# JuliaControl/ModelPredictiveControl.jl

Measured on AMD Instinct MI355X. Metric: QP solves/sec (moveinput!), higher is better.
Workload: dtype f64

## Files before the change

### modelpredictivecontrol.jl_amd/csrc/mpcqp_bodies.h

```cpp
#pragma once
#include <math.h>

#include <type_traits>

#include "mpcqp_types.h"

#if defined(MPCQP_PROFILE) && defined(__HIP_DEVICE_COMPILE__)
#define MPCQP_TIC() const long long tic_ = clock64()
#define MPCQP_TOC(i) prof_[i] += (double)(clock64() - tic_)
#define MPCQP_TICK(name) const long long name = clock64()
#define MPCQP_TOCK(i, name) prof_[i] += (double)(clock64() - name)
#elif defined(MPCQP_ISA_MARKERS) && defined(__HIP_DEVICE_COMPILE__)
#define MPCQP_MARK_(txt) do { __builtin_amdgcn_sched_barrier(0); asm volatile("; MPCQP_MARK " txt ::: "memory"); __builtin_amdgcn_sched_barrier(0); } while (0)
#define MPCQP_TIC() MPCQP_MARK_("tic")
#define MPCQP_TOC(i) MPCQP_MARK_("toc " #i)
#define MPCQP_TICK(name) MPCQP_MARK_("tic " #name)
#define MPCQP_TOCK(i, name) MPCQP_MARK_("toc " #i)
#define MPCQP_MTIC() MPCQP_MARK_("tic")
#define MPCQP_MTOC(name) MPCQP_MARK_("toc " name)
#else
#define MPCQP_TIC() ((void)0)
#define MPCQP_TOC(i) ((void)0)
#define MPCQP_TICK(name) ((void)0)
#define MPCQP_TOCK(i, name) ((void)0)
#endif
#ifndef MPCQP_MTIC
#define MPCQP_MTIC() ((void)0)
#define MPCQP_MTOC(name) ((void)0)
#endif

#ifndef MPCQP_POLISH_FACTS
#define MPCQP_POLISH_FACTS 1
#endif
#ifndef MPCQP_POLISH_BUDGET
#define MPCQP_POLISH_BUDGET 3
#endif
#ifndef MPCQP_POLISH_MU
#define MPCQP_POLISH_MU 1e-7
#endif
#ifndef MPCQP_POLISH_RP
#define MPCQP_POLISH_RP 1e-6
#endif
#ifndef MPCQP_EAPPLY44_HCMAX
#define MPCQP_EAPPLY44_HCMAX 10
#endif
#ifndef MPCQP_EAPPLY44_UNROLL
#define MPCQP_EAPPLY44_UNROLL 2
#endif
#ifndef MPCQP_EV_UNROLL
#if defined(MPCQP_STEP_WAVES) && MPCQP_STEP_WAVES == 1
#define MPCQP_EV_UNROLL 16
#else
#define MPCQP_EV_UNROLL 4
#endif
#endif
#define MPCQP_PRAGMA_(x) _Pragma(#x)
#define MPCQP_PRAGMA(x) MPCQP_PRAGMA_(x)
#ifndef MPCQP_ETDE_UNROLL
#if defined(MPCQP_STEP_WAVES) && MPCQP_STEP_WAVES == 1
#define MPCQP_ETDE_UNROLL 4
#else
#define MPCQP_ETDE_UNROLL 2
#endif
#endif
#ifndef MPCQP_ETDE_VREG_MAX
#define MPCQP_ETDE_VREG_MAX 32
#endif
#ifndef MPCQP_ETDE_VREG_CHUNK
#define MPCQP_ETDE_VREG_CHUNK 2
#endif
#ifndef MPCQP_SOLVEBIG_UNROLL
#if defined(MPCQP_STEP_WAVES) && MPCQP_STEP_WAVES == 1
#define MPCQP_SOLVEBIG_UNROLL 8
#else
#define MPCQP_SOLVEBIG_UNROLL 2
#endif
#endif
#ifndef MPCQP_HZ_UNROLL
#define MPCQP_HZ_UNROLL 4
#endif
#ifndef MPCQP_PANEL_UNROLL
#define MPCQP_PANEL_UNROLL 16
#endif
#ifndef MPCQP_URMW_UNROLL
#define MPCQP_URMW_UNROLL 4
#endif
#ifndef MPCQP_SPEC_DENSE
#define MPCQP_SPEC_DENSE 0
#endif
#ifndef MPCQP_SPEC_NW
#define MPCQP_SPEC_NW 0
#endif
#ifndef MPCQP_ETAPPLY_NB
#define MPCQP_ETAPPLY_NB 3
#endif

namespace mpcqp {

MPCQP_HD inline double rcp(double x) {
#if defined(__HIP_DEVICE_COMPILE__)
    const double r = __builtin_amdgcn_rcp(x);
    return fma(fma(-x, r, 1.0), r, r);
#else
    return 1.0 / x;
#endif
}

MPCQP_HD inline double rcp_fast(double x) {
#if defined(__HIP_DEVICE_COMPILE__)
    return __builtin_amdgcn_rcp(x);
#else
    return 1.0 / x;
#endif
}

MPCQP_HD inline double fmx(double a, double b) {
#if defined(__HIP_DEVICE_COMPILE__)
    double r;
    asm("v_max_f64 %0, %1, %2" : "=v"(r) : "v"(a), "v"(b));
    return r;
#else
    return fmax(a, b);
#endif
}
MPCQP_HD inline double fmn(double a, double b) {
#if defined(__HIP_DEVICE_COMPILE__)
    double r;
    asm("v_min_f64 %0, %1, %2" : "=v"(r) : "v"(a), "v"(b));
    return r;
#else
    return fmin(a, b);
#endif
}
MPCQP_HD inline double fmx_abs(double a, double b) {
#if defined(__HIP_DEVICE_COMPILE__)
    double r;
    asm("v_max_f64 %0, %1, |%2|" : "=v"(r) : "v"(a), "v"(b));
    return r;
#else
    return fmax(a, fabs(b));
#endif
}

template <int NU, int NY, int NXH, int HP, int HC, int NEPS, unsigned GMASK, int DNB = 1>
struct StaticDims {
    static constexpr bool is_static = true;
    static constexpr int nu = NU, ny = NY, nxh = NXH, Hp = HP, Hc = HC, neps = NEPS;
    static constexpr int nDU = NU * HC, nZ = NU * HC + NEPS, nU = NU * HP, nY = NY * HP;
    static constexpr int npk = pk_size(nZ);
    static constexpr int nw = MPCQP_SPEC_NW, nW = MPCQP_SPEC_NW * (HP + 1);
    static constexpr int sp = (NY * NU) % 16 == 0 ? NY * NU + 8 : NY * NU;
    static constexpr int rs = (NY == 4 && NU == 4) ? 6 : NU;
    static constexpr uint32_t gmask = GMASK;
    static constexpr int default_nb = DNB;
    static constexpr int zpad = DNB == 1 ? HC - 1 : 0;
    int B, nd, nD, max_iter;
    double gap_tol, res_tol, dual_reg;
    uint32_t flags;
    MPCQP_HD static constexpr int eps_host() { return eps_host_group(GMASK, NEPS); }
    MPCQP_HD static constexpr int len(int p) {
        return p == P_BOX ? nZ : p == P_U ? nDU : p == P_DU ? nDU : p == P_Y ? nY : p == P_X ? nxh : p == P_W ? nW : 0;
    }
    MPCQP_HD static constexpr int cnt(int p) { return len(p) + ((p == P_Y && eps_host() >= 0) ? 1 : 0); }
    MPCQP_HD static constexpr int rowoff(int g) {
        int o = 0;
        for (int i = 0; i < g; ++i)
            if ((GMASK >> i) & 1u) o += cnt(i >> 1);
        return o;
    }
    MPCQP_HD static constexpr int nrows() { return rowoff(NGROUP); }
    MPCQP_HD explicit StaticDims(const Dims& d)
        : B(d.B), nd(d.nd), nD(d.nD), max_iter(d.max_iter), gap_tol(d.gap_tol), res_tol(d.res_tol),
          dual_reg(d.dual_reg), flags(d.flags) {}
    static bool matches_dims(const Dims& d) {
        return d.nu == NU && d.ny == NY && d.nxh == NXH && d.Hp == HP && d.Hc == HC &&
               d.neps == NEPS && d.default_nb == DNB && d.nw == MPCQP_SPEC_NW;
    }
    static bool matches(const Dims& d) { return matches_dims(d) && d.gmask == GMASK; }
};

template <class DM>
constexpr bool has_w() {
    if constexpr (DM::is_static) return DM::nw > 0;
    else return true;
}

constexpr int NROWARR = 7;

struct Carve {
    int S, Phi, zero, z, dz, q, zlo, zhi, gt, rd, dinv, zb, xh, F, tA[NPAIR], tB[NPAIR], ucum, exT, Wm;
    int rows[NROWARR];
    int jl, blk;
    int total;
};

template <class DM>
MPCQP_HD constexpr bool one_row_per_lane() {
    if constexpr (DM::is_static) return DM::nZ <= WAVE;
    else return false;
}

template <class W, class DM>
MPCQP_HD constexpr bool phi_layout() {
#if defined(__HIP_DEVICE_COMPILE__)
    if constexpr (DM::is_static) return DM::nZ <= WAVE && W::NTEAM == 1;
    else return false;
#else
    return false;
#endif
}
template <class W, class DM>
MPCQP_HD constexpr int phi_ix(int i, int j) {
    if constexpr (phi_layout<W, DM>()) return phi(DM::nZ, i, j);
    else return pk(i, j);
}

template <class DM>
MPCQP_HD constexpr int hwq_() {
    if constexpr (DM::is_static) {
        constexpr int n = (DM::nY + WAVE - 1) / WAVE;
        return (DM::nZ <= WAVE && n <= 4) ? n : 0;
    } else {
        return 0;
    }
}

template <class DM>
MPCQP_HD inline int stride_S(const DM& d) {
    if constexpr (DM::is_static) return DM::sp;
    else return d.ny * d.nu;
}

template <class DM>
MPCQP_HD inline int zpad_S(const DM&) {
    if constexpr (DM::is_static) return DM::zpad;
    else return 0;
}

template <class DM>
MPCQP_HD inline int rowstride_S(const DM& d) {
    if constexpr (DM::is_static) return DM::rs;
    else return d.nu;
}

template <class DM>
MPCQP_HD inline Carve make_carve(const DM& d) {
    Carve c{};
    int o = 0;
    auto take = [&](int n) { int r = o; o += (n + 1) & ~1; return r; };
    c.S = take((d.Hp + zpad_S(d)) * stride_S(d));
    c.Phi = take(d.npk);
    c.zero = take(6);
    c.z = take(d.nZ); c.dz = take(d.nZ); c.q = take(d.nZ);
    c.gt = take(d.nZ); c.rd = take(d.nZ);
    c.dinv = take(d.nZ > WAVE ? d.nZ : 0);
    c.xh = take(d.nxh);
    c.zb = take((DM::is_static && d.nZ <= WAVE) ? 0 : d.nZ);
    c.zlo = c.dz; c.zhi = c.gt;
    c.F = -1;
    MPCQP_UNROLL
    for (int p = 0; p < NPAIR; ++p) {
        const bool won = (d.gmask >> (2 * P_W)) & 3u;
        const bool on = ((d.gmask >> (2 * p)) & 3u) || (won && (p == P_Y || p == P_U));
        c.tA[p] = take((on || p == P_Y) ? d.cnt(p) : 0);
        c.tB[p] = take((on && p != P_BOX) ? d.cnt(p) : 0);
    }
    c.F = (((d.gmask >> (2 * P_Y)) & 3u) && c.tB[P_Y] >= 0) ? c.tB[P_Y] : take(d.nY);
    c.ucum = take(d.nDU);
    c.Wm = take(((d.gmask >> (2 * P_W)) & 3u) ? d.nw * (d.ny + d.nu) : 0);
    c.exT = take(((d.gmask >> (2 * P_X)) & 3u) ? d.Hc * d.nxh * d.nu : 0);
    const int M = DM::is_static ? 0 : d.nrows();
    MPCQP_UNROLL
    for (int a = 0; a < NROWARR; ++a) c.rows[a] = take(M);
    c.jl = take(d.default_nb ? 0 : (d.Hc + 2) / 2 + 1);
    c.blk = take(d.default_nb ? 0 : (d.Hp + 1) / 2 + 1);
    c.total = o;
    return c;
}

template <class W>
MPCQP_HD constexpr bool team_mine_mfma(int idx) {
    if (W::NTEAM == 1) return true;
    return (idx + 1) % W::NTEAM == W::WV;
}
template <class W>
MPCQP_HD constexpr bool team_any_mfma(int count) {
    for (int i = 0; i < count; ++i)
        if (team_mine_mfma<W>(i)) return true;
    return false;
}

template <class DM>
MPCQP_HD constexpr bool setup_prefetch() {
    if constexpr (DM::is_static) {
        return DM::nZ <= WAVE && DM::Hc < WAVE && DM::Hp <= WAVE && DM::nxh <= WAVE && DM::nu <= 16 && (DM::nY + WAVE - 1) / WAVE <= 4 &&
               (DM::Hp * DM::ny * DM::nu + WAVE - 1) / WAVE <= 16 && DM::nw == 0 && !MPCQP_SPEC_DENSE;
    } else {
        return false;
    }
}

template <class DM, bool ON = setup_prefetch<DM>()>
struct SetupLoads {
    static constexpr bool on = false;
    template <class W>
    MPCQP_HD void issue(const W&, const DM&, const Model&, const StepIO&, int) {}
};

template <class DM>
struct SetupLoads<DM, true> {
    static constexpr bool on = true;
    static constexpr int NS = (DM::Hp * DM::ny * DM::nu + WAVE - 1) / WAVE;
    static constexpr int QY = (DM::nY + WAVE - 1) / WAVE;
    static constexpr bool KREG = QY * DM::nxh <= 48;
    double S[NS];
    int jl, blk;
    double x0, lu[DM::nu], luc, zw;
    double Bv[QY], K[KREG ? QY : 1][KREG ? DM::nxh : 1], Ry[QY], Md[QY];
    double sc[SC_N];
    double du[4];
    double Y0[2][QY];
    double Nd, Cw;

    template <int Q>
    MPCQP_HD static double pick(const double (&a)[Q], int k) {
        double v = a[0];
        MPCQP_UNROLL
        for (int q_ = 1; q_ < Q; ++q_) v = (k >= WAVE * q_) ? a[q_] : v;
        return v;
    }

    template <class W>
    MPCQP_HD void issue(const W& w, const DM& d, const Model& m, const StepIO& io, int b) {
        constexpr int ns = DM::Hp * DM::ny * DM::nu, nY = DM::nY, nDU = DM::nDU, nx = DM::nxh, nu = DM::nu, ny = DM::ny, n = DM::nZ;
        const int lane = w.lane;
        MPCQP_UNROLL
        for (int q_ = 0; q_ < NS; ++q_) { const int i = lane + WAVE * q_; S[q_] = m.Stab[(size_t)b * ns + (i < ns ? i : 0)]; }
        jl = 0; blk = 0;
        if (!d.default_nb) { jl = m.jl[lane <= DM::Hc ? lane : 0]; blk = m.blk[lane < DM::Hp ? lane : 0]; }
        x0 = io.xhat0[(size_t)b * nx + (lane < nx ? lane : 0)];
        MPCQP_UNROLL
        for (int cc = 0; cc < nu; ++cc) lu[cc] = io.lastu0[(size_t)b * nu + cc];
        luc = io.lastu0[(size_t)b * nu + lane % nu];
        const bool rconst = d.flags & 1u;
        MPCQP_UNROLL
        for (int q_ = 0; q_ < QY; ++q_) {
            const int r = lane + WAVE * q_, rc = r < nY ? r : 0;
            Bv[q_] = m.Bvec[(size_t)b * nY + rc];
            if constexpr (KREG) {
                MPCQP_UNROLL
                for (int k = 0; k < nx; ++k) K[q_][k] = m.Ktab[(size_t)b * nx * nY + (size_t)k * nY + rc];
            }
        }
        MPCQP_UNROLL
        for (int q_ = 0; q_ < QY; ++q_) {
            const int r = lane + WAVE * q_, rc = r < nY ? r : 0;
            Ry[q_] = io.Ry[rconst ? (size_t)b * ny + (rc % ny) : (size_t)b * nY + rc];
            Md[q_] = m.Mdiag[(size_t)b * nY + rc];
        }
        const int kc = lane < nDU ? lane : 0;
        const double* anyk = m.Ndiag + (size_t)b * nDU + kc;
        MPCQP_UNROLL
        for (int a = 0; a < SC_N; ++a) sc[a] = *(m.stepc ? m.stepc + ((size_t)b * SC_N + a) * nDU + kc : anyk);
        du[0] = *(m.DUmin ? m.DUmin + (size_t)b * nDU + kc : anyk);
        du[1] = *(m.DUmax ? m.DUmax + (size_t)b * nDU + kc : anyk);
        du[2] = *((d.neps && m.C_dumin) ? m.C_dumin + (size_t)b * nDU + kc : anyk);
        du[3] = *((d.neps && m.C_dumax) ? m.C_dumax + (size_t)b * nDU + kc : anyk);
        MPCQP_UNROLL
        for (int q_ = 0; q_ < QY; ++q_) {
            const int r = lane + WAVE * q_, rc = r < nY ? r : 0;
            const double* anyr = m.Mdiag + (size_t)b * nY + rc;
            Y0[0][q_] = *(m.Y0min ? m.Y0min + (size_t)b * nY + rc : anyr);
            Y0[1][q_] = *(m.Y0max ? m.Y0max + (size_t)b * nY + rc : anyr);
        }
        Nd = *anyk;
        Cw = d.neps ? m.Cwt[b] : 0.0;
        zw = io.Z[(size_t)b * n + (lane < nDU - nu ? lane + nu : (lane >= nDU && lane < n) ? lane : 0)];
        MPCQP_SCHED_FENCE();
    }
};

template <class W, class DM>
struct Qp {
    W& w;
    const DM& d;
    const Model& m;
    const int b;
    double* sm;
    Carve c;
    int *jlt, *blkt;
    double *S, *Phi;
    int sp;
    int rs;

    MPCQP_HD Qp(W& w_, const DM& d_, const Model& m_, int b_, double* sm_)
        : w(w_), d(d_), m(m_), b(b_), sm(sm_), c(make_carve(d_)), sp(stride_S(d_)), rs(rowstride_S(d_)) {
        jlt = reinterpret_cast<int*>(sm + c.jl);
        blkt = reinterpret_cast<int*>(sm + c.blk);
        S = sm + c.S + zpad_S(d_) * sp;
        Phi = sm + c.Phi;
    }

    MPCQP_HD static void load4q(const double* p, double* x) {
#if defined(__HIP_DEVICE_COMPILE__)
        typedef double v2q_ __attribute__((ext_vector_type(2)));
        const v2q_ a = reinterpret_cast<const v2q_*>(p)[0], b2 = reinterpret_cast<const v2q_*>(p)[1];
        x[0] = a.x; x[1] = a.y; x[2] = b2.x; x[3] = b2.y;
#else
        x[0] = p[0]; x[1] = p[1]; x[2] = p[2]; x[3] = p[3];
#endif
    }

    MPCQP_HD bool pair_on(int p) const { return (d.gmask >> (2 * p)) & 3u; }
    MPCQP_HD bool group_on(int g) const { return (d.gmask >> g) & 1u; }
    MPCQP_HD int jl(int j) const { return d.default_nb ? j : jlt[j]; }
    MPCQP_HD int blk(int t) const { return d.default_nb ? (t < d.Hc - 1 ? t : d.Hc - 1) : blkt[t]; }

    template <class Fn>
    MPCQP_HD void stage(const double* g, int n, Fn dst) {
        constexpr int NB = 8;
        for (int i0 = 0; i0 < n; i0 += NB * WAVE) {
            double v[NB];
            MPCQP_UNROLL
            for (int q_ = 0; q_ < NB; ++q_) { const int i = i0 + w.lane + WAVE * q_; v[q_] = g[i < n ? i : 0]; }
            MPCQP_UNROLL
            for (int q_ = 0; q_ < NB; ++q_) { const int i = i0 + w.lane + WAVE * q_; if (i < n) dst(i, v[q_]); }
        }
    }

    MPCQP_HD void load_tables() { load_tables(SetupLoads<DM, false>{}); }
    template <class PRE>
    MPCQP_HD void load_tables(const PRE& pre) {
        const int nb_ = d.ny * d.nu, ns = d.Hp * nb_;
        auto putS = [&](int i, double v) {
            const int blk_ = i / nb_, e = i - blk_ * nb_, a = e / d.nu;
            S[blk_ * sp + a * rs + (e - a * d.nu)] = v;
        };
        if constexpr (PRE::on) {
            MPCQP_UNROLL
            for (int q_ = 0; q_ < PRE::NS; ++q_) { const int i = w.lane + WAVE * q_; if (i < ns) putS(i, pre.S[q_]); }
        } else {
            stage(m.Stab + (size_t)b * ns, ns, putS);
        }
        for (int i = w.lane; i < zpad_S(d) * sp; i += WAVE) sm[c.S + i] = 0.0;
        if (!d.default_nb) {
            if constexpr (PRE::on) {
                if (w.lane <= d.Hc) jlt[w.lane] = pre.jl;
                if (w.lane < d.Hp) blkt[w.lane] = pre.blk;
            } else {
                for (int i = w.lane; i <= d.Hc; i += WAVE) jlt[i] = m.jl[i];
                for (int i = w.lane; i < d.Hp; i += WAVE) blkt[i] = m.blk[i];
            }
        }
        if (pair_on(P_X) && m.exT) {
            const int ne = d.Hc * d.nxh * d.nu;
            stage(m.exT + (size_t)b * ne, ne, [&](int i, double v) { sm[c.exT + i] = v; });
        }
        if constexpr (has_w<DM>()) {
            if (pair_on(P_W)) {
                const int n1 = d.nw * d.ny, n2 = d.nw * d.nu;
                for (int i = w.lane; i < n1; i += WAVE) sm[c.Wm + i] = m.Wy[(size_t)b * n1 + i];
                for (int i = w.lane; i < n2; i += WAVE) sm[c.Wm + n1 + i] = m.Wu[(size_t)b * n2 + i];
            }
        }
        if (w.lane < 4) sm[c.zero + w.lane] = 0.0;
        w.sync();
    }

    MPCQP_HD double Wy_(int i, int a) const { return sm[c.Wm + i + d.nw * a]; }
    MPCQP_HD double Wu_(int i, int cc) const { return sm[c.Wm + d.nw * d.ny + i + d.nw * cc]; }
    MPCQP_HD int blkW(int t) const { return blk(t < d.Hp ? t : d.Hp - 1); }
    MPCQP_HD double Ew_at(int t, int i, int j, int cc) const {
        double g = 0.0;
        if (t >= 1 && t - 1 >= jl(j)) {
            const double* Sb = S + (t - 1 - jl(j)) * sp + cc;
            for (int a = 0; a < d.ny; ++a) g += Wy_(i, a) * Sb[a * rs];
        }
        if (j <= blkW(t)) g += Wu_(i, cc);
        return g;
    }
    MPCQP_HD void W_fold(const double* wW, double* tY, bool freshY, double* tU, bool freshU) {
        const int nw = d.nw, ny = d.ny, nu = d.nu;
        for (int r = w.lane; r < d.nY; r += WAVE) {
            const int t = r / ny, a = r - t * ny;
            double acc = freshY ? 0.0 : tY[r];
            for (int i = 0; i < nw; ++i) acc += Wy_(i, a) * wW[(t + 1) * nw + i];
            tY[r] = acc;
        }
        for (int k = w.lane; k < d.nDU; k += WAVE) {
            const int j = k / nu, cc = k - j * nu;
            const int t1 = (j + 1 < d.Hc) ? jl(j + 1) : d.Hp + 1;
            double acc = freshU ? 0.0 : tU[k];
            for (int t = jl(j); t < t1; ++t)
                for (int i = 0; i < nw; ++i) acc += Wu_(i, cc) * wW[t * nw + i];
            tU[k] = acc;
        }
        w.sync();
    }

    MPCQP_HD double block_prefix(double x) {
#if defined(__HIP_DEVICE_COMPILE__)
        if constexpr (DM::is_static) {
            if constexpr (DM::nu == 4 && DM::nDU <= WAVE) {
                x += W::template dpp<0x114>(x);
                x += W::template dpp<0x118>(x);
                const int row = w.lane >> 4, cc = w.lane & 3;
                double carry = 0.0;
                MPCQP_UNROLL
                for (int rr = 1; rr <= (DM::Hc - 1) / 4; ++rr) {
                    const double y = w.fetch(x, ((row - rr) << 4) + 12 + cc);
                    carry += row >= rr ? y : 0.0;
                }
                return x + carry;
            }
        }
#endif
        const int nu = d.nu, j = w.lane / nu;
        for (int s_ = 1; s_ < d.Hc; s_ <<= 1) {
            const double y = w.fetch(x, w.lane - s_ * nu);
            x += (j >= s_ && w.lane < d.nDU) ? y : 0.0;
        }
        return x;
    }
    MPCQP_HD double block_suffix(double x) {
#if defined(__HIP_DEVICE_COMPILE__)
        if constexpr (DM::is_static) {
            if constexpr (DM::nu == 4 && DM::nDU <= WAVE) {
                x += W::template dpp<0x104>(x);
                x += W::template dpp<0x108>(x);
                const int row = w.lane >> 4, cc = w.lane & 3;
                double carry = 0.0;
                MPCQP_UNROLL
                for (int rr = 1; rr <= (DM::Hc - 1) / 4; ++rr) {
                    const double y = w.fetch(x, ((row + rr) << 4) + cc);
                    carry += row + rr < 4 ? y : 0.0;
                }
                return x + carry;
            }
        }
#endif
        const int nu = d.nu, j = w.lane / nu;
        for (int s_ = 1; s_ < d.Hc; s_ <<= 1) {
            const double y = w.fetch(x, w.lane + s_ * nu);
            x += (j + s_ < d.Hc && w.lane < d.nDU) ? y : 0.0;
        }
        return x;
    }

    MPCQP_HD void E_apply(const double* v, double* out) {
        if constexpr (W::NTEAM > 1) { static_assert(W::WV == 0, MPCQP_POST_WV0); w.post(TJ_EV, (int)(v - sm), (int)(out - sm)); }
        E_apply_share(v, out);
        if constexpr (W::NTEAM > 1) w.join();
    }
    MPCQP_HD void E_apply_share(const double* v, double* out) { E_apply_share_<false>(v, out, nullptr); }
    MPCQP_HD static constexpr int ev_slots() {
        if constexpr (DM::is_static) {
            constexpr bool c3 = DM::nu == 4 && DM::nY <= 2 * WAVE && DM::Hc <= MPCQP_EAPPLY44_HCMAX;
            constexpr int nr = (DM::nY + WAVE - 1) / WAVE;
            return (W::NTEAM == 1 && DM::default_nb && (c3 || DM::zpad > 0) && nr <= 4) ? nr : 0;
        } else {
            return 0;
        }
    }
    template <bool REG>
    MPCQP_HD void E_apply_share_(const double* v, double* out, double* mine_q) {
        const int ny = d.ny, nu = d.nu;
        if constexpr (DM::is_static) {
            if (W::NTEAM == 1 && DM::nu == 4 && DM::nY <= 2 * WAVE && DM::Hc <= MPCQP_EAPPLY44_HCMAX && d.default_nb) {
                const int r0 = w.lane, r1 = w.lane + WAVE;
                const bool ok0 = r0 < DM::nY, ok1 = r1 < DM::nY;
                const int t0 = (ok0 ? r0 : 0) / DM::ny, a0 = (ok0 ? r0 : 0) % DM::ny;
                const int t1 = (ok1 ? r1 : 0) / DM::ny, a1 = (ok1 ? r1 : 0) % DM::ny;
                const double* Sa = S + t0 * sp + a0 * rs;
                const double* Sb = S + t1 * sp + a1 * rs;
                double x0 = 0.0, x1 = 0.0, y0 = 0.0, y1 = 0.0;
                MPCQP_PRAGMA(unroll MPCQP_EAPPLY44_UNROLL)
                for (int j = 0; j < DM::Hc; ++j) {
                    double vv[4], sa[4], sb[4];
                    load4q(v + j * 4, vv);
                    load4q(Sa - j * DM::sp, sa);
                    load4q(Sb - j * DM::sp, sb);
                    x0 = fma(sa[0], vv[0], x0); x1 = fma(sa[1], vv[1], x1);
                    y0 = fma(sb[0], vv[0], y0); y1 = fma(sb[1], vv[1], y1);
                    x0 = fma(sa[2], vv[2], x0); x1 = fma(sa[3], vv[3], x1);
                    y0 = fma(sb[2], vv[2], y0); y1 = fma(sb[3], vv[3], y1);
                    if (j % MPCQP_EAPPLY44_UNROLL == MPCQP_EAPPLY44_UNROLL - 1) MPCQP_SCHED_FENCE();
                }
                if (ok0) out[r0] = x0 + x1;
                if (ok1) out[r1] = y0 + y1;
                if constexpr (REG) {
                    mine_q[0] = x0 + x1;
                    if constexpr (DM::nY > WAVE) mine_q[1] = y0 + y1;
                }
                return;
            }
        }
#if defined(__HIP_DEVICE_COMPILE__)
        if constexpr (DM::is_static) {
            if (DM::zpad > 0 && d.default_nb) {
                constexpr int NR = (DM::nY + WAVE - 1) / WAVE;
                auto mine = [](int q_) { return (q_ + 1) % W::NTEAM == W::WV; };
                const double* Sa[NR];
                double acc[NR][2];
                MPCQP_UNROLL
                for (int q_ = 0; q_ < NR; ++q_) {
                    const int r = w.lane + WAVE * q_;
                    const int rr = r < DM::nY ? r : 0;
                    Sa[q_] = S + (rr / DM::ny) * DM::sp + (rr % DM::ny) * DM::rs;
                    acc[q_][0] = acc[q_][1] = 0.0;
                }
                if constexpr (W::NTEAM == 1 || (W::WV == 0 ? NR >= W::NTEAM : NR >= W::WV)) {
                MPCQP_PRAGMA(unroll MPCQP_EV_UNROLL)
                for (int j = 0; j < DM::Hc; ++j) {
                    MPCQP_UNROLL
                    for (int cc = 0; cc < DM::nu; ++cc) {
                        const double vv = v[j * DM::nu + cc];
                        MPCQP_UNROLL
                        for (int q_ = 0; q_ < NR; ++q_)
                            if (mine(q_)) acc[q_][cc & 1] = fma(Sa[q_][cc - j * DM::sp], vv, acc[q_][cc & 1]);
                    }
                }
                }
                MPCQP_UNROLL
                for (int q_ = 0; q_ < NR; ++q_) {
                    const int r = w.lane + WAVE * q_;
                    if (mine(q_) && r < DM::nY) out[r] = acc[q_][0] + acc[q_][1];
                    if constexpr (REG) mine_q[q_] = acc[q_][0] + acc[q_][1];
                }
                return;
            }
        }
#endif
        if constexpr (W::WV != 0) return;
        for (int r = w.lane; r < d.nY; r += WAVE) {
            const int t = r / ny, a = r - t * ny;
            double acc0 = 0.0;
            for (int j = 0; j < d.Hc && jl(j) <= t; ++j) {
                const double* Sb = S + (t - jl(j)) * sp + a * rs;
                const double* vj = v + j * nu;
                for (int cc = 0; cc < nu; ++cc) acc0 += Sb[cc] * vj[cc];
            }
            out[r] = acc0;
        }
    }

    MPCQP_HD void Et_apply_add(const double* wv, double* out, double scale = 1.0, int t_hi = -1) {
        if constexpr (W::NTEAM > 1) { static_assert(W::WV == 0, MPCQP_POST_WV0); w.post(TJ_ETW, (int)(wv - sm), (int)(out - sm), t_hi, 0, scale); }
        Et_apply_share(wv, out, scale, t_hi);
        if constexpr (W::NTEAM > 1) w.join();
    }
    MPCQP_HD void Et_apply_share(const double* wv, double* out, double scale, int t_hi) {
        double none = 0.0;
        Et_apply_share_<false>(wv, out, scale, t_hi, none);
    }
    template <bool REG>
    MPCQP_HD void Et_apply_share_(const double* wv, double* out, double scale, int t_hi, double& mine_k) {
        const int ny = d.ny, nu = d.nu;
        if (t_hi < 0) t_hi = d.Hp;
        if constexpr (DM::is_static) {
            if (W::NTEAM == 1 && DM::ny == 4 && DM::nu == 4 && DM::nDU <= WAVE && d.default_nb) {
                const int k = w.lane < DM::nDU ? w.lane : 0;
                const int j = k >> 2, a = k & 3;
                const double* Sb = S - j * sp + a * rs;
                const double* wa = wv + a;
                double p0 = 0.0, p1 = 0.0, p2 = 0.0, p3 = 0.0;
                constexpr int NB = MPCQP_ETAPPLY_NB, NBAT = (DM::Hp + NB - 1) / NB;
                double sr[2][NB][4], wt[2][NB];
                auto ld = [&](int bt, int buf) {
                    MPCQP_UNROLL
                    for (int u = 0; u < NB; ++u) {
                        const int t = bt * NB + u;
                        if (t >= DM::Hp) break;
                        load4q(Sb + t * DM::sp, sr[buf][u]);
                        wt[buf][u] = wa[t * 4];
                    }
                };
                ld(0, 0);
                MPCQP_UNROLL
                for (int bt = 0; bt < NBAT; ++bt) {
                    if (bt * NB >= t_hi) break;
                    const int buf = bt & 1;
                    if (bt + 1 < NBAT) ld(bt + 1, buf ^ 1);
                    MPCQP_SCHED_FENCE();
                    MPCQP_UNROLL
                    for (int u = 0; u < NB; ++u) {
                        const int t = bt * NB + u;
                        if (t >= DM::Hp) break;
                        const double wv_ = t < t_hi ? wt[buf][u] : 0.0;
                        p0 = fma(sr[buf][u][0], wv_, p0); p1 = fma(sr[buf][u][1], wv_, p1);
                        p2 = fma(sr[buf][u][2], wv_, p2); p3 = fma(sr[buf][u][3], wv_, p3);
                    }
                    MPCQP_SCHED_FENCE();
                }
                p0 = w.quad_sum(p0); p1 = w.quad_sum(p1); p2 = w.quad_sum(p2); p3 = w.quad_sum(p3);
                const double mine = a == 0 ? p0 : a == 1 ? p1 : a == 2 ? p2 : p3;
                if constexpr (REG) { if (w.lane < DM::nDU) mine_k += scale * mine; }
                else { if (w.lane < DM::nDU) out[k] += scale * mine; }
                return;
            }
        }
#if defined(__HIP_DEVICE_COMPILE__)
        if constexpr (DM::is_static) {
            if (DM::zpad > 0 && d.default_nb) {
                constexpr int NQ = (DM::nDU + WAVE - 1) / WAVE;
                auto mine = [](int q_) { return (q_ + 1) % W::NTEAM == W::WV; };
                const double* Sk[NQ];
                double acc[NQ][2];
                MPCQP_UNROLL
                for (int q_ = 0; q_ < NQ; ++q_) {
                    const int k = w.lane + WAVE * q_;
                    const int kk = k < DM::nDU ? k : 0;
                    Sk[q_] = S - (kk / DM::nu) * DM::sp + (kk % DM::nu);
                    acc[q_][0] = acc[q_][1] = 0.0;
                }
                if constexpr (W::NTEAM == 1 || (W::WV == 0 ? NQ >= W::NTEAM : NQ >= W::WV)) {
                MPCQP_PRAGMA(unroll MPCQP_EV_UNROLL)
                for (int t = 0; t < DM::Hp; ++t) {
                    if (t >= t_hi) break;
                    MPCQP_UNROLL
                    for (int a = 0; a < DM::ny; ++a) {
                        const double wt = wv[t * DM::ny + a];
                        MPCQP_UNROLL
                        for (int q_ = 0; q_ < NQ; ++q_)
                            if (mine(q_)) acc[q_][a & 1] = fma(Sk[q_][t * DM::sp + a * DM::rs], wt, acc[q_][a & 1]);
                    }
                }
                }
                MPCQP_UNROLL
                for (int q_ = 0; q_ < NQ; ++q_) {
                    const int k = w.lane + WAVE * q_;
                    if constexpr (REG) { if (k < DM::nDU) mine_k += scale * (acc[q_][0] + acc[q_][1]); }
                    else { if (mine(q_) && k < DM::nDU) out[k] += scale * (acc[q_][0] + acc[q_][1]); }
                }
                return;
            }
        }
#endif
        if constexpr (W::WV != 0) return;
        for (int k = w.lane; k < d.nDU; k += WAVE) {
            const int j = k / nu, cc = k - j * nu, t0 = jl(j);
            const double* Sk = S + cc;
            double acc0 = 0.0, acc1 = 0.0;
            MPCQP_UNROLL4
            for (int t = 0; t < t_hi; ++t) {
                const bool ok = t >= t0;
                const double* Sb = Sk + (ok ? t - t0 : 0) * sp;
                const double* wt = wv + t * ny;
                double p0 = 0.0, p1 = 0.0;
                int a = 0;
                for (; a + 1 < ny; a += 2) { p0 += Sb[a * rs] * wt[a]; p1 += Sb[(a + 1) * rs] * wt[a + 1]; }
                if (a < ny) p0 += Sb[a * rs] * wt[a];
                acc0 += ok ? p0 : 0.0;
                acc1 += ok ? p1 : 0.0;
            }
            if constexpr (REG) mine_k += scale * (acc0 + acc1);
            else out[k] += scale * (acc0 + acc1);
        }
    }

    MPCQP_HD static void unpack_idx(int idx, int& i, int& ip) {
        i = (int)((sqrt(8.0 * idx + 1.0) - 1.0) * 0.5);
        while (i * (i + 1) / 2 > idx) --i;
        while ((i + 1) * (i + 2) / 2 <= idx) ++i;
        ip = idx - i * (i + 1) / 2;
    }

#if defined(__HIP_DEVICE_COMPILE__)
    typedef double v4d __attribute__((ext_vector_type(4)));
    template <int I0, int NT, class F>
    static __device__ __forceinline__ void etde_passes(F& f) {
        if constexpr (I0 < NT) {
            f(std::integral_constant<int, I0>{});
            etde_passes<(I0 == 0 ? 2 : I0 + 1), NT>(f);
        }
    }
    template <bool PH = false, bool MK = false>
    __device__ __forceinline__ int EtDE_add_mfma(const double* dd, double* P, double scale, const double* tb,
                                                 const double* Hg = nullptr, bool ow = false) {
        if constexpr (W::NTEAM > 1) { static_assert(W::WV == 0, MPCQP_POST_WV0); w.post(TJ_ETDE, (int)(dd - sm), (int)(P - sm), tb ? (int)(tb - sm) : 0, (ow ? 1 : 0) | (Hg ? 2 : 0) | (tb ? 4 : 0), scale); }
        const int e = EtDE_share<PH, MK && W::NTEAM == 1>(dd, P, scale, tb ? tb : dd, Hg, ow, tb != nullptr);
        if constexpr (W::NTEAM > 1) w.join();
        return e;
    }
    template <bool PH = false, bool MK = false>
    __device__ __forceinline__ int EtDE_share(const double* dd, double* P, double scale, const double* tb, const double* Hg, bool ow, bool has_tb) {
        return EtDE_share_<PH, MK>(dd, P, scale, tb, Hg, ow, has_tb);
    }
    template <bool PH, bool MK = false>
    __device__ __forceinline__ int EtDE_share_(const double* dd, double* P, double scale, const double* tb, const double* Hg, bool ow, bool has_tb) {
        static_assert(!PH || phi_layout<W, DM>(), "column-block-major Phi outside its kernels");
        ow = ow || Hg != nullptr;
        constexpr int NU = DM::nu, NY = DM::ny, NDU = DM::nDU, NYR = DM::nY, SP = DM::sp, RS = DM::rs;
        constexpr int NT = (NDU + 15) / 16, NK = (NYR + 3) / 4;
        const int li = w.lane & 15, lk = w.lane >> 4;
        constexpr bool MSK = MK && NK <= WAVE;
        bool knz = false;
        if constexpr (MSK) {
            MPCQP_UNROLL
            for (int u = 0; u < 4; ++u) {
                const int r = 4 * w.lane + u, rr = r < NYR ? r : 0;
                knz = knz || (r < NYR && (dd[rr] != 0.0 || (has_tb && tb[rr] != 0.0)));
            }
        }
        const int lkp = (NY % 4 == 0) ? (((lk & 1) << 1) | (lk >> 1)) : lk;
        int offI[NT], offL[NT], jI[NT];
        MPCQP_UNROLL
        for (int I = 0; I < NT; ++I) {
            const int i = 16 * I + li;
            const int j = i / NU, cc = i - j * NU;
            const int tj = jl(i < NDU ? j : 0);
            jI[I] = i < NDU ? tj : (1 << 20);
            offI[I] = -tj * SP + cc;
            offL[I] = offI[I] + lkp * RS;
        }
        constexpr int IE = NDU / 16, LE = NDU % 16;
        int eps_t0 = -1;
        if (DM::neps && has_tb && IE < NT) {
            int v = (jl((16 * IE) / NU) * NY) / 4;
            v = v < NK ? v : NK;
            if ((4 * v) % NY != 0) v = 0;
            eps_t0 = (4 * v) / NY;
        }
        constexpr int QK = NY % 4 == 0 ? NY / 4 : 1;
        constexpr int DJ = (16 % NU == 0) ? QK * (16 / NU) : 1;
        constexpr bool VREG = NY % 4 == 0 && 16 % NU == 0 && DM::zpad > 0 && DM::zpad >= 16 / NU - 1 &&
                              NK <= MPCQP_ETDE_VREG_MAX;
        double V[VREG ? NK : 1];
        if constexpr (VREG) {
            const int cbv = li / NU, civ = li - cbv * NU;
            const double* Vb = S - cbv * SP + lkp * RS + civ;
            MPCQP_UNROLL
            for (int k = 0; k < NK; ++k) V[k] = Vb[(k / QK) * SP + 4 * (k % QK) * RS];
        }
        auto pass = [&](auto I0c) {
            constexpr int I0 = decltype(I0c)::value;
            if constexpr (W::NTEAM > 1) {
                if constexpr (!team_mine_mfma<W>(I0 == 0 ? 0 : I0 - 1)) return;
            }
            constexpr int MAXT = NT + 1;
            constexpr int I1 = (I0 == 0 && NT > 1) ? 1 : I0;
            v4d acc[2][MAXT];
            MPCQP_UNROLL
            for (int x = 0; x < 2; ++x) {
                MPCQP_UNROLL
                for (int J = 0; J < MAXT; ++J) acc[x][J] = v4d{0.0, 0.0, 0.0, 0.0};
            }
            const bool erow = DM::neps && has_tb && IE >= I0 && IE <= I1;
            auto entry_ok = [&](int I, int J, int reg) {
                const bool eI = erow && I == IE;
                const int il = 4 * reg + lk;
                const bool rowok = 16 * I + 15 < NDU || 16 * I + il < NDU;
                const bool colok = 16 * J + 15 < NDU || 16 * J + li < NDU;
                const bool low = J < I || li <= il;
                return colok && ((rowok && low) || (eI && il == LE));
            };
            auto entry_idx_pk = [&](int I, int J, int reg) {
                const int G = 4 * I + reg;
                return 8 * G * (G + 1) + 16 * J + 4 * (G + 1) * lk + li;
            };
            int eb[MAXT];
            auto entry_base = [&]() {
                if constexpr (PH) {
                    const int q_ = li >> 2;
                    const int eb0 = 4 * q_ * (DM::nZ - 2 - 2 * q_) + (li & 3) + 4 * lk;
                    MPCQP_UNROLL
                    for (int J = 0; J <= I1; ++J) eb[J] = eb0 + 16 * J * (DM::nZ - 2 - 8 * J) - 64 * J * q_;
                }
            };
            auto entry_idx = [&](int I, int J, int reg) {
                if constexpr (PH) return eb[J] + 64 * I + 16 * reg;
                else return entry_idx_pk(I, J, reg);
            };
            double hreg[2][MAXT][4];
            auto hload = [&]() {
                MPCQP_UNROLL
                for (int I = I0; I <= I1; ++I) {
                    MPCQP_UNROLL
                    for (int J = 0; J <= I; ++J) {
                        MPCQP_UNROLL
                        for (int reg = 0; reg < 4; ++reg)
                            hreg[I - I0][J][reg] = Hg[entry_ok(I, J, reg) ? (unsigned)entry_idx_pk(I, J, reg) : 0u];
                    }
                }
            };
            constexpr bool LATEH = !VREG && NT > 4;
            if (Hg && !VREG && !LATEH) hload();
            auto kfirst = [&](int I) {
                int v = (jl((16 * I) / NU) * NY) / 4;
                v = v < NK ? v : NK;
                if (erow && I == IE) { if ((4 * v) % NY != 0) v = 0; }
                return v;
            };
            const int kB = (I1 > I0) ? kfirst(I1) : NK;
            const int kA = kfirst(I0) < kB ? kfirst(I0) : kB;
            unsigned klo = ~0u, khi = ~0u;
            if constexpr (MSK) {
                const int k0 = VREG ? ((DJ * I0 < NK) ? DJ * I0 : NK) : kA;
                const unsigned long long km = __builtin_amdgcn_ballot_w64(knz && w.lane >= k0);
                klo = (unsigned)km;
                khi = (unsigned)(km >> 32);
            }
            auto kon = [&](int kk) { return !MSK || (((kk < 32 ? klo : khi) >> (kk & 31)) & 1u) != 0; };
            const int zoff = (int)((sm + c.zero) - S);
            struct Ops { double dv, tbv, e[NT]; };
            auto kload = [&](int kk, Ops& o) {
                o.tbv = 0.0;
                if constexpr (NY % 4 == 0) {
                    const int t = (4 * kk) / NY, a0 = 4 * kk - t * NY;
                    const int base = t * SP + a0 * RS;
                    o.dv = dd[4 * kk + lkp];
                    if (erow) o.tbv = tb[4 * kk + lkp];
                    MPCQP_UNROLL
                    for (int J = 0; J <= I1; ++J) o.e[J] = S[(DM::zpad || t >= jI[J]) ? base + offL[J] : zoff];
                } else {
                    const int r = 4 * kk + lk;
                    const bool rok = r < NYR;
                    const int rr = rok ? r : 0;
                    const int t = rr / NY, a = rr - t * NY;
                    o.dv = rok ? dd[rr] : 0.0;
                    if (erow) o.tbv = rok ? tb[rr] : 0.0;
                    const int base = t * SP + a * RS;
                    MPCQP_UNROLL
                    for (int J = 0; J <= I1; ++J) o.e[J] = S[(rok && (DM::zpad || t >= jI[J])) ? base + offI[J] : zoff];
                }
            };
            auto kcomp = [&](const Ops& o, bool row0, bool row1) {
                MPCQP_UNROLL
                for (int I = I0; I <= I1; ++I) {
                    if (I == I0 ? !row0 : !row1) continue;
                    const bool eI = erow && I == IE;
                    double ad = o.e[I] * o.dv;
                    if (eI && li == LE) ad = o.tbv;
                    MPCQP_UNROLL
                    for (int J = 0; J <= I; ++J)
                        acc[I - I0][J] = __builtin_amdgcn_mfma_f64_16x16x4f64(ad, o.e[J], acc[I - I0][J], 0, 0, 0);
                }
            };
            if constexpr (VREG) {
                constexpr int kA_ = (DJ * I0 < NK) ? DJ * I0 : NK;
                constexpr int kB_ = (I1 > I0) ? ((DJ * I1 < NK) ? DJ * I1 : NK) : NK;
                constexpr int CH = MPCQP_ETDE_VREG_CHUNK;
                constexpr bool EP = DM::neps != 0 && IE >= I0 && IE <= I1;
                double dvb[2][CH], tbb[2][EP ? CH : 1];
                const double* ddl = dd + lkp;
                const double* tbl = tb + lkp;
                auto ldc = [&](int c0, int buf) {
                    MPCQP_UNROLL
                    for (int u = 0; u < CH; ++u) {
                        const int kk = c0 + u;
                        if (kk >= NK) break;
                        dvb[buf][u] = ddl[4 * kk];
                        if constexpr (EP) { if (erow) tbb[buf][u] = tbl[4 * kk]; }
                    }
                };
                if constexpr (MSK) {
                    if (Hg) hload();
                    MPCQP_UNROLL
                    for (int kk = kA_; kk < NK; ++kk) {
                        if (!kon(kk)) continue;
                        const double dv = ddl[4 * kk];
                        double tbv = 0.0;
// ... 2915 lines not shown
```

### modelpredictivecontrol.jl_amd/csrc/mpcqp_devwave.h

```cpp
#pragma once
#include <hip/hip_runtime.h>

#include <cstdlib>

#include "mpcqp_types.h"

#ifndef MPCQP_STEP_WAVES
#define MPCQP_STEP_WAVES 2
#endif

namespace mpcqp {

struct DevWave {
    int lane;
    static constexpr int NTEAM = 1, WV = 0;
    __device__ __forceinline__ void post(int, int = 0, int = 0, int = 0, int = 0, double = 0.0) {}
    __device__ __forceinline__ void join() {}
    __device__ __forceinline__ void sync() {
        __builtin_amdgcn_fence(__ATOMIC_RELEASE, "wavefront");
        __builtin_amdgcn_wave_barrier();
        __builtin_amdgcn_fence(__ATOMIC_ACQUIRE, "wavefront");
    }

    __device__ __forceinline__ void sync_lds() {
        asm volatile("s_waitcnt lgkmcnt(0)" ::: "memory");
        __builtin_amdgcn_wave_barrier();
    }

    template <int CTRL>
    static __device__ __forceinline__ double dpp(double v) {
        int lo = __double2loint(v), hi = __double2hiint(v);
        lo = __builtin_amdgcn_update_dpp(0, lo, CTRL, 0xf, 0xf, true);
        hi = __builtin_amdgcn_update_dpp(0, hi, CTRL, 0xf, 0xf, true);
        return __hiloint2double(hi, lo);
    }
    static __device__ __forceinline__ double lane_value(double v, int src) {
        const int lo = __builtin_amdgcn_readlane(__double2loint(v), src);
        const int hi = __builtin_amdgcn_readlane(__double2hiint(v), src);
        return __hiloint2double(hi, lo);
    }
    template <int CTRL, int ROWMASK>
    static __device__ __forceinline__ double dpp_rows(double v, double old) {
        int lo = __builtin_amdgcn_update_dpp(__double2loint(old), __double2loint(v), CTRL, ROWMASK, 0xf, false);
        int hi = __builtin_amdgcn_update_dpp(__double2hiint(old), __double2hiint(v), CTRL, ROWMASK, 0xf, false);
        return __hiloint2double(hi, lo);
    }
    template <bool SELF, class Op>
    static __device__ __forceinline__ double reduce(double v, Op op) {
        v = op(v, dpp<0xB1>(v));
        v = op(v, dpp<0x4E>(v));
        v = op(v, dpp<0x141>(v));
        v = op(v, dpp<0x140>(v));
        v = op(v, dpp_rows<0x142, 0xA>(v, SELF ? v : 0.0));
        v = op(v, dpp_rows<0x143, 0xC>(v, SELF ? v : 0.0));
        return lane_value(v, 63);
    }
    __device__ __forceinline__ double quad_sum(double v) {
        v += dpp<0xB1>(v);
        v += dpp<0x4E>(v);
        return v;
    }
    __device__ __forceinline__ double sum(double v) { return reduce<false>(v, [](double x, double y) { return x + y; }); }
    static __device__ __forceinline__ double mn_(double x, double y) { double r; asm("v_min_f64 %0, %1, %2" : "=v"(r) : "v"(x), "v"(y)); return r; }
    static __device__ __forceinline__ double mx_(double x, double y) { double r; asm("v_max_f64 %0, %1, %2" : "=v"(r) : "v"(x), "v"(y)); return r; }
    __device__ __forceinline__ double minv(double v) { return reduce<true>(v, [](double x, double y) { return mn_(x, y); }); }
    __device__ __forceinline__ double maxv(double v) { return reduce<true>(v, [](double x, double y) { return mx_(x, y); }); }
    __device__ __forceinline__ int isum(int v) {
#pragma unroll
        for (int o = 32; o > 0; o >>= 1) v += __shfl_xor(v, o, 64);
        return v;
    }
    __device__ __forceinline__ double bcast(double v, int src) { return lane_value(v, src); }
    __device__ __forceinline__ void relane() { asm volatile("" : "+v"(lane)); }
    __device__ __forceinline__ double fetch(double v, int src) const {
        const int lo = __builtin_amdgcn_ds_bpermute(src << 2, __double2loint(v));
        const int hi = __builtin_amdgcn_ds_bpermute(src << 2, __double2hiint(v));
        return __hiloint2double(hi, lo);
    }
    __device__ __forceinline__ bool any(bool p) { return __builtin_amdgcn_ballot_w64(p) != 0; }
    template <int K, int ROWS, bool REV>
    static __device__ __forceinline__ void chain4(double& r, double c0, double c1, double c2, double c3) {
        if constexpr (!REV)
            asm("s_nop 1\n\t"
                "v_fmac_f64_dpp %0, %0, %1 row_newbcast:%5 row_mask:%9 bank_mask:0xf\n\t"
                "s_nop 1\n\t"
                "v_fmac_f64_dpp %0, %0, %2 row_newbcast:%6 row_mask:%9 bank_mask:0xf\n\t"
                "s_nop 1\n\t"
                "v_fmac_f64_dpp %0, %0, %3 row_newbcast:%7 row_mask:%9 bank_mask:0xf\n\t"
                "s_nop 1\n\t"
                "v_fmac_f64_dpp %0, %0, %4 row_newbcast:%8 row_mask:%9 bank_mask:0xf"
                : "+v"(r)
                : "v"(c0), "v"(c1), "v"(c2), "v"(c3), "n"(K), "n"(K + 1), "n"(K + 2), "n"(K + 3), "n"(ROWS));
        else
            asm("s_nop 1\n\t"
                "v_fmac_f64_dpp %0, %0, %4 row_newbcast:%8 row_mask:%9 bank_mask:0xf\n\t"
                "s_nop 1\n\t"
                "v_fmac_f64_dpp %0, %0, %3 row_newbcast:%7 row_mask:%9 bank_mask:0xf\n\t"
                "s_nop 1\n\t"
                "v_fmac_f64_dpp %0, %0, %2 row_newbcast:%6 row_mask:%9 bank_mask:0xf\n\t"
                "s_nop 1\n\t"
                "v_fmac_f64_dpp %0, %0, %1 row_newbcast:%5 row_mask:%9 bank_mask:0xf"
                : "+v"(r)
                : "v"(c0), "v"(c1), "v"(c2), "v"(c3), "n"(K), "n"(K + 1), "n"(K + 2), "n"(K + 3), "n"(ROWS));
    }
    template <int C>
    static __device__ __forceinline__ double rowbc(double v) { return __builtin_amdgcn_update_dpp(0.0, v, 0x150 + C, 0xf, 0xf, true); }
    template <int L, bool NOP>
    static __device__ __forceinline__ void rowbc_fms(double& a, double x, double y) {
        if constexpr (NOP)
            asm("s_nop 1\n\tv_fmac_f64_dpp %0, %1, -%2 row_newbcast:%3 row_mask:0xf bank_mask:0xf" : "+v"(a) : "v"(x), "v"(y), "n"(L));
        else
            asm("v_fmac_f64_dpp %0, %1, -%2 row_newbcast:%3 row_mask:0xf bank_mask:0xf" : "+v"(a) : "v"(x), "v"(y), "n"(L));
    }
    template <int K, int ROWS>
    static __device__ __forceinline__ void fmabc4(double& acc, double x, double c0, double c1, double c2, double c3) {
        asm("s_nop 1\n\t"
            "v_fmac_f64_dpp %0, %1, %2 row_newbcast:%6 row_mask:%10 bank_mask:0xf\n\t"
            "v_fmac_f64_dpp %0, %1, %3 row_newbcast:%7 row_mask:%10 bank_mask:0xf\n\t"
            "v_fmac_f64_dpp %0, %1, %4 row_newbcast:%8 row_mask:%10 bank_mask:0xf\n\t"
            "v_fmac_f64_dpp %0, %1, %5 row_newbcast:%9 row_mask:%10 bank_mask:0xf"
            : "+v"(acc)
            : "v"(x), "v"(c0), "v"(c1), "v"(c2), "v"(c3), "n"(K), "n"(K + 1), "n"(K + 2), "n"(K + 3), "n"(ROWS));
    }
};

extern __shared__ __attribute__((aligned(16))) double mpcqp_smem[];

template <int T, int WV_>
struct DevWaveT : DevWave {
    static constexpr int NTEAM = T, WV = WV_;
    double* mbox;
    __device__ __forceinline__ void post(int job, int a0 = 0, int a1 = 0, int a2 = 0, int a3 = 0, double sc = 0.0) {
        if (lane == 0) {
            int* mi = reinterpret_cast<int*>(mbox);
            mi[0] = job; mi[1] = a0; mi[2] = a1; mi[3] = a2; mi[4] = a3;
            mbox[3] = sc;
        }
        __syncthreads();
    }
    __device__ __forceinline__ void join() { __syncthreads(); }
};

template <class SD>
__global__ __launch_bounds__(64) __attribute__((amdgpu_waves_per_eu(2, 8))) void k_hessian_s(Dims d, Model m) {
    DevWave w{(int)threadIdx.x};
    const SD sd(d);
    hessian_body(w, sd, m, (int)blockIdx.x, mpcqp_smem);
}

template <class SD>
__global__ __launch_bounds__(64) __attribute__((amdgpu_waves_per_eu(MPCQP_STEP_WAVES, 8))) void k_step_s(Dims d, Model m, StepIO io) {
    DevWave w{(int)threadIdx.x};
    const SD sd(d);
    step_body(w, sd, m, io, (int)blockIdx.x, mpcqp_smem);
}

template <class DM> constexpr int auto_team();

template <class SD, int T, int WV>
__device__ __forceinline__ void team_run(int wv, int lane, double* mbox, const SD& sd, const Model& m, const StepIO& io) {
#if defined(__HIP_DEVICE_COMPILE__)
    if constexpr (WV < T) {
        if (wv == WV) {
            DevWaveT<T, WV> w;
            w.lane = lane; w.mbox = mbox;
            if constexpr (WV == 0) { step_body(w, sd, m, io, (int)blockIdx.x, mpcqp_smem); w.post(TJ_EXIT); }
            else team_helper(w, sd, m, (int)blockIdx.x, mpcqp_smem);
        } else {
            team_run<SD, T, WV + 1>(wv, lane, mbox, sd, m, io);
        }
    }
#endif
}
template <class SD, int T>
__global__ __launch_bounds__(64 * T) __attribute__((amdgpu_waves_per_eu(1, 8))) void k_step_team(Dims d, Model m, StepIO io) {
    const SD sd(d);
    const int wv = __builtin_amdgcn_readfirstlane((int)threadIdx.x >> 6);
    double* mbox = mpcqp_smem + make_carve(sd).total;
    team_run<SD, T, 0>(wv, (int)threadIdx.x & 63, mbox, sd, m, io);
}
#ifndef MPCQP_TEAM
#define MPCQP_TEAM 0
#endif

inline hipError_t ensure_lds(const void* fn, size_t bytes) {
    if (bytes <= 64 * 1024) return hipSuccess;
    return hipFuncSetAttribute(fn, hipFuncAttributeMaxDynamicSharedMemorySize, (int)bytes);
}

template <class SD>
inline hipError_t launch_step_static(const Dims& d, const Model& m, const StepIO& io, hipStream_t st) {
    size_t lds = (size_t)make_carve(SD(d)).total * sizeof(double);
    if (const char* pad = getenv("MPCQP_LDS_PAD")) lds += (size_t)atoi(pad);
    constexpr int T = MPCQP_TEAM > 0 ? MPCQP_TEAM : auto_team<SD>();
    if constexpr (T > 1) {
        lds += 8 * sizeof(double);
        hipError_t e = ensure_lds((const void*)k_step_team<SD, T>, lds);
        if (e != hipSuccess) return e;
        hipLaunchKernelGGL((k_step_team<SD, T>), dim3(d.B), dim3(WAVE * T), lds, st, d, m, io);
        return hipGetLastError();
    } else {
        hipError_t e = ensure_lds((const void*)k_step_s<SD>, lds);
        if (e != hipSuccess) return e;
        hipLaunchKernelGGL(k_step_s<SD>, dim3(d.B), dim3(WAVE), lds, st, d, m, io);
        return hipGetLastError();
    }
}

template <class SD>
inline hipError_t launch_hessian_static(const Dims& d, const Model& m, hipStream_t st) {
    const size_t lds = (size_t)make_carve(SD(d)).total * sizeof(double);
    hipError_t e = ensure_lds((const void*)k_hessian_s<SD>, lds);
    if (e != hipSuccess) return e;
    hipLaunchKernelGGL(k_hessian_s<SD>, dim3(d.B), dim3(WAVE), lds, st, d, m);
    return hipGetLastError();
}

}
```

### modelpredictivecontrol.jl_amd/csrc/mpcqp_types.h

```cpp
#pragma once
#include <stdint.h>

#if defined(__HIPCC__)
#define MPCQP_HD __host__ __device__ __attribute__((always_inline))
#define MPCQP_UNROLL _Pragma("unroll")
#define MPCQP_UNROLL4 _Pragma("unroll 4")
#define MPCQP_NOUNROLL _Pragma("nounroll")
#if defined(__HIP_DEVICE_COMPILE__)
#define MPCQP_SCHED_FENCE() __builtin_amdgcn_sched_barrier(0)
#else
#define MPCQP_SCHED_FENCE() ((void)0)
#endif
#else
#define MPCQP_SCHED_FENCE() ((void)0)
#define MPCQP_HD
#define MPCQP_UNROLL
#define MPCQP_UNROLL4
#define MPCQP_NOUNROLL
#endif

#define MPCQP_KERNEL_REV 17

namespace mpcqp {

enum TeamJob { TJ_EXIT = 0, TJ_ETDE = 1, TJ_PANEL = 2, TJ_EV = 3, TJ_ETW = 4, TJ_UROWS = 5, TJ_WROWS = 6, TJ_XROWS = 7, TJ_PANELROWS = 8, TJ_LOADH = 9, TJ_HZ = 10 };
#define MPCQP_POST_WV0 "only wavefront 0 of a team posts jobs: a helper that reached this call would wait at the barrier for ever"


enum { P_BOX = 0, P_U = 1, P_DU = 2, P_Y = 3, P_X = 4, P_W = 5, NPAIR = 6, NGROUP = 12 };

constexpr int WAVE = 64;
constexpr double BIG = 1e300;

MPCQP_HD constexpr int eps_host_group(uint32_t gmask, int neps) {
    return !neps ? -1 : ((gmask >> (2 * P_Y + 1)) & 1u) ? 2 * P_Y + 1 : ((gmask >> (2 * P_Y)) & 1u) ? 2 * P_Y : -1;
}

struct Dims {
    int B, nxh, nu, ny, nd, Hp, Hc, neps;
    int nZ, nDU, nU, nY, nD;
    int nw, nW;
    int npk;
    uint32_t gmask;
    int rowoff_[NGROUP + 1];
    int cnt_[NPAIR];
    int default_nb;
    int dense_w;
    int max_iter;
    double gap_tol, res_tol, dual_reg;
    uint32_t flags;
    static constexpr bool is_static = false;
    MPCQP_HD int cnt(int p) const { return cnt_[p]; }
    MPCQP_HD int len(int p) const { return p == P_Y ? nY : cnt_[p]; }
    MPCQP_HD int eps_host() const { return eps_host_group(gmask, neps); }
    MPCQP_HD int rowoff(int g) const { return rowoff_[g]; }
    MPCQP_HD int nrows() const { return rowoff_[NGROUP]; }
};

struct Model {
    const double *Ahat, *Bu, *C, *Bd, *Dd, *dop;
    double* Stab;
    double* Ktab;
    double* Bvec;
    double* Gdtab;
    double* exT;
    double* kxT;
    double* bxv;
    double* Xdtab;
    double* Hpk;
    const double *Mdiag, *Ndiag, *Ldiag, *Cwt;
    const double* Mblk;
    const double* Mfull;
    const double* Ndense;
    const double* Ldense;
    const double *U0min, *U0max, *DUmin, *DUmax, *Y0min, *Y0max, *x0min, *x0max;
    const double *C_umin, *C_umax, *C_dumin, *C_dumax, *C_ymin, *C_ymax, *c_x0min, *c_x0max;
    const double *Wy, *Wu, *Wd, *Wr;
    const double* w_op;
    const double* ry_now;
    const double *Wmin, *Wmax, *C_wmin, *C_wmax;
    const int* jl;
    const int* blk;
    const double* stepc;
};
enum { SC_UMIN = 0, SC_UMAX = 1, SC_LSUM = 2, SC_LNZ = 3, SC_N = 4 };

struct KfParams {
    const double* Khat;
    const int* i_ym;
    int nym;
};

struct StepIO {
    const double *xhat0, *lastu0, *Ry, *Ru, *d0, *Dhat0;
    double *Z, *u0, *Yhat0;
    int32_t *status, *iters;
    double *q_keep, *F_keep;
    const double* lam_prev;
    double* lam_out;
    double *prof;
    double *audit;
    const double* kf_K;
    const int* kf_iym;
    const double* kf_y0m;
    double* xhat0_out;
    int kf_nym, kf_predict;
    int kf_late;
};

MPCQP_HD constexpr int pk(int i, int j) { return 4 * ((i >> 2) + 1) * (2 * (i >> 2) + (i & 3)) + j; }
MPCQP_HD constexpr int pk_size(int n) { return pk(n, 0); }

MPCQP_HD constexpr int phi_blk(int n, int c) { return 4 * c * n - 8 * c * (c - 1); }
MPCQP_HD constexpr int phi_col(int n, int j) { return 4 * (j >> 2) * (n - 2 * (j >> 2) - 2) + (j & 3); }
MPCQP_HD constexpr int phi(int n, int i, int j) { return phi_col(n, j) + 4 * i; }
constexpr bool phi_bijective(int n) {
    const int G = (n + 3) / 4, size = pk_size(n);
    if (phi_blk(n, G) != size) return false;
    bool seen[pk_size(64)] = {};
    int cnt = 0;
    for (int c = 0; c < G; ++c) {
        if (phi_col(n, 4 * c) < 0 || phi_col(n, 4 * c) != phi_blk(n, c) - 16 * c) return false;
        for (int i = 4 * c; i < n; ++i)
            for (int j = 4 * c; j < 4 * c + 4; ++j) {
                const int s = phi(n, i, j);
                if (s < 0 || s >= size || seen[s]) return false;
                if (s != phi_blk(n, c) + 4 * (i - 4 * c) + (j & 3)) return false;
                seen[s] = true;
                ++cnt;
            }
    }
    return cnt == size;
}
template <int N>
struct PhiProof {
    static_assert(phi_bijective(N), "phi(n, i, j) is not a bijection onto [0, pk_size(n))");
    static constexpr bool ok = PhiProof<N - 1>::ok;
};
template <>
struct PhiProof<0> { static constexpr bool ok = true; };
static_assert(PhiProof<64>::ok, "column-block-major layout of Phi, n = 1 .. 64");

}
```

Measured before the change: 4.966 million.

## Restructure Et_apply for ny=nu=4 with per-lane scalar loads and permlane reduction

Adds a device-only specialised path for Et_apply with static ny=nu=4 dims. Lanes are remapped so each lane loads single doubles of S and w from LDS into a register array and accumulates a few partial sums over time-shifted columns. The partials are combined across lanes with permlane32/permlane16 swaps instead of per-lane quad loads. This aims to cut LDS traffic and serial FMA chains, at the cost of more registers (full Hp-length arrays) and a new dependency on the zpad layout and the newer permlane-swap intrinsics.

```diff
diff --git a/modelpredictivecontrol.jl_amd/csrc/mpcqp_bodies.h b/modelpredictivecontrol.jl_amd/csrc/mpcqp_bodies.h
--- a/modelpredictivecontrol.jl_amd/csrc/mpcqp_bodies.h
+++ b/modelpredictivecontrol.jl_amd/csrc/mpcqp_bodies.h
@@ -93,6 +93,9 @@
 #endif
 #ifndef MPCQP_ETAPPLY_NB
 #define MPCQP_ETAPPLY_NB 3
+#endif
+#ifndef MPCQP_ETW_NB
+#define MPCQP_ETW_NB 4
 #endif
 
 namespace mpcqp {
@@ -657,6 +660,64 @@
     MPCQP_HD void Et_apply_share_(const double* wv, double* out, double scale, int t_hi, double& mine_k) {
         const int ny = d.ny, nu = d.nu;
         if (t_hi < 0) t_hi = d.Hp;
+#if defined(__HIP_DEVICE_COMPILE__)
+        if constexpr (DM::is_static) {
+            if constexpr (W::NTEAM == 1 && DM::ny == 4 && DM::nu == 4 && DM::nDU <= WAVE && DM::default_nb != 0 && DM::zpad >= 3) {
+                int ln = w.lane;
+                asm volatile("" : "+v"(ln));
+                const int li = ln & 15, lk = ln >> 4;
+                const int a = ((lk & 1) << 1) | (lk >> 1);
+                const double* Xb = S - (li >> 2) * DM::sp + a * DM::rs + (li & 3);
+                const double* wa = wv + a;
+                constexpr int NT = (DM::nDU + 15) / 16;
+                constexpr int NB = MPCQP_ETW_NB, NBAT = (DM::Hp + NB - 1) / NB;
+                double X[DM::Hp], wt[DM::Hp];
+                double acc[4] = {0.0, 0.0, 0.0, 0.0};
+                auto lds_b64 = [](const double* p) { return *(const volatile __attribute__((address_space(3))) double*)p; };
+                auto ld = [&](int bt) {
+                    MPCQP_UNROLL
+                    for (int u = 0; u < NB; ++u) {
+                        const int t = bt * NB + u;
+                        if (t >= DM::Hp) break;
+                        X[t] = lds_b64(Xb + t * DM::sp);
+                        wt[t] = lds_b64(wa + t * 4);
+                    }
+                };
+                ld(0);
+                MPCQP_UNROLL
+                for (int bt = 0; bt < NBAT; ++bt) {
+                    if (bt * NB >= t_hi) break;
+                    if (bt + 1 < NBAT) ld(bt + 1);
+                    MPCQP_SCHED_FENCE();
+                    MPCQP_UNROLL
+                    for (int u = 0; u < NB; ++u) {
+                        const int t = bt * NB + u;
+                        if (t >= DM::Hp) break;
+                        const double wv_ = t < t_hi ? wt[t] : 0.0;
+                        MPCQP_UNROLL
+                        for (int J = 0; J < NT; ++J)
+                            if (t - 4 * J >= 0) acc[J] = fma(X[t - 4 * J], wv_, acc[J]);
+                    }
+                    MPCQP_SCHED_FENCE();
+                }
+                double r02 = acc[0], y02 = acc[NT > 2 ? 2 : 0];
+                W::swap32(r02, y02);
+                r02 += y02;
+                double r13 = r02;
+                if constexpr (NT > 1) {
+                    double y13 = acc[NT > 3 ? 3 : 1];
+                    r13 = acc[1];
+                    W::swap32(r13, y13);
+                    r13 += y13;
+                }
+                W::swap16(r02, r13);
+                const double mine = r02 + r13;
+                if constexpr (REG) { if (w.lane < DM::nDU) mine_k += scale * mine; }
+                else { if (w.lane < DM::nDU) out[w.lane] += scale * mine; }
+                return;
+            }
+        }
+#endif
         if constexpr (DM::is_static) {
             if (W::NTEAM == 1 && DM::ny == 4 && DM::nu == 4 && DM::nDU <= WAVE && d.default_nb) {
                 const int k = w.lane < DM::nDU ? w.lane : 0;
diff --git a/modelpredictivecontrol.jl_amd/csrc/mpcqp_devwave.h b/modelpredictivecontrol.jl_amd/csrc/mpcqp_devwave.h
--- a/modelpredictivecontrol.jl_amd/csrc/mpcqp_devwave.h
+++ b/modelpredictivecontrol.jl_amd/csrc/mpcqp_devwave.h
@@ -59,6 +59,18 @@
         v += dpp<0xB1>(v);
         v += dpp<0x4E>(v);
         return v;
+    }
+    static __device__ __forceinline__ void swap32(double& x, double& y) {
+        const auto lo = __builtin_amdgcn_permlane32_swap(__double2loint(x), __double2loint(y), false, false);
+        const auto hi = __builtin_amdgcn_permlane32_swap(__double2hiint(x), __double2hiint(y), false, false);
+        x = __hiloint2double(hi[0], lo[0]);
+        y = __hiloint2double(hi[1], lo[1]);
+    }
+    static __device__ __forceinline__ void swap16(double& x, double& y) {
+        const auto lo = __builtin_amdgcn_permlane16_swap(__double2loint(x), __double2loint(y), false, false);
+        const auto hi = __builtin_amdgcn_permlane16_swap(__double2hiint(x), __double2hiint(y), false, false);
+        x = __hiloint2double(hi[0], lo[0]);
+        y = __hiloint2double(hi[1], lo[1]);
     }
     __device__ __forceinline__ double sum(double v) { return reduce<false>(v, [](double x, double y) { return x + y; }); }
     static __device__ __forceinline__ double mn_(double x, double y) { double r; asm("v_min_f64 %0, %1, %2" : "=v"(r) : "v"(x), "v"(y)); return r; }
diff --git a/modelpredictivecontrol.jl_amd/csrc/mpcqp_types.h b/modelpredictivecontrol.jl_amd/csrc/mpcqp_types.h
--- a/modelpredictivecontrol.jl_amd/csrc/mpcqp_types.h
+++ b/modelpredictivecontrol.jl_amd/csrc/mpcqp_types.h
@@ -19,7 +19,7 @@
 #define MPCQP_NOUNROLL
 #endif
 
-#define MPCQP_KERNEL_REV 17
+#define MPCQP_KERNEL_REV 18
 
 namespace mpcqp {
 
```

Result: faster. 5.171 million (median of 6 runs) (+4.1%).
